# aws/sagemaker-xgboost-container

Hardware: NVIDIA H100
Metric: boosting rounds/sec (higher is better)
Workload: dtype int64

## Files before the change

### sagemaker-xgboost-container_b200/csrc/grow.cu

```cuda
#include "grow.h"
#include <algorithm>
#include <cmath>
#include <cstdlib>
#include <cstring>
#include "comm.h"

namespace b200 {

__global__ void pack_tree_kernel(TreeArrays t, const int* n_nodes, DevNode* out, int cap) {
  const int nn = *n_nodes;
  for (int i = blockIdx.x * blockDim.x + threadIdx.x; i < cap; i += gridDim.x * blockDim.x) {
    DevNode d;
    if (i < nn) { d.cond = t.split_cond[i]; d.left = t.left[i]; d.right = t.right[i]; d.fidx_dl = (unsigned)t.split_index[i] | ((unsigned)t.default_left[i] << 31); }
    else { d.cond = 0.f; d.left = -1; d.right = -1; d.fidx_dl = 0; }
    out[i] = d;
  }
}
__global__ void snapshot_h_kernel(const GH64* slot, long long* cache, size_t entries) {
  for (size_t e = (size_t)blockIdx.x * blockDim.x + threadIdx.x; e < entries; e += (size_t)gridDim.x * blockDim.x) cache[e] = slot[e].h;
}
__global__ void slot_from_cache_kernel(GH64* slot, const long long* cache, size_t entries) {
  for (size_t e = (size_t)blockIdx.x * blockDim.x + threadIdx.x; e < entries; e += (size_t)gridDim.x * blockDim.x) { GH64 v; v.g = 0; v.h = cache[e]; slot[e] = v; }
}
__global__ void gather_u32_kernel(const unsigned* src, const unsigned* idx, unsigned* dst, int64_t n) {
// ... 44 lines not shown
  if (lg_iters > 0) {
    max_nodes = 2 * lg_iters + 1; max_level_nodes = 2; region = 0;
    pool_slots = (size_t)lg_iters + kLgFirstFreeSlot;
  } else {
    max_nodes = (1 << (max_depth + 1)) - 1; max_level_nodes = 1 << (max_depth - 1); region = max_level_nodes;
    pool_slots = 2 * (size_t)region;
  }
  cap_nodes = (max_nodes + 15) & ~15;
  slot_stride = hist_slot_entries(ngroups, tw);
  const size_t partial_entries = hist_partial_entries(ngroups, tw, engine_num_sms(), max_level_nodes);
  const size_t pool_bytes = pool_slots * slot_stride * sizeof(GH64) + partial_entries * sizeof(int2);
  size_t free_b = 0, total_b = 0; cudaMemGetInfo(&free_b, &total_b);
  B200_CHECK(pool_bytes < free_b / 2 + hist_pool.n * sizeof(GH64) + hist_partials.n * sizeof(int2),
             "histogram pool for this max_depth / max_leaves / feature count does not fit in device memory");
  hist_pool.alloc(pool_slots * slot_stride);
  hist_partials.alloc(partial_entries);
  gpair.alloc((size_t)gp_stride * K + 512); gpair.zero(s); err.alloc(1); tree_index_dev.alloc(1);
  if (!leaf_scale.p) { leaf_scale.alloc(1); set_leaf_scale(1.0f); }
  root_h_cache.alloc(slot_stride);
  const bool routed = routes(lg_iters, max_depth);
  for (int i = 0; i < 2; ++i) { const size_t m = i == 0 || !routed ? (size_t)n : 0; ridx[i].alloc(m); gp[i].alloc(m); tl[i].alloc(tail_pos ? m : 0); }
  route_tiles = routed ? (unsigned)((n + kRouteTile - 1) / kRouteTile) : 0u;
  node_of_row.alloc(routed ? (size_t)n : 0);
  route_counts.alloc(routed && max_depth >= 2 ? ((size_t)1 << (max_depth - 2)) * route_tiles : 0);
  max_tiles = (unsigned)((n + kPartTile - 1) / kPartTile) + max_level_nodes + 1;
  scratch.alloc(3 * (size_t)max_level_nodes + 8);
  state_block.alloc(carve(gs, 0)); state_block.zero(s);
  carve(gs, (uintptr_t)state_block.p);
  tree_block.alloc(tree_block_bytes(cap_nodes));
  const TreeBlock tb = tree_block_layout(tree_block.p, cap_nodes);
  gs.n_nodes = tb.n_nodes; ta = tb.t; packed.alloc(cap_nodes);
  ic_path.alloc(n_ic ? (size_t)cap_nodes * F : 0); ic_allowed.alloc(n_ic ? (size_t)cap_nodes * F : 0);
  ic_sets.alloc((size_t)n_ic * F); ic_sets_host.clear();
  hist_configure();
  global_n = n;
  if (Comm::get().distributed()) {
    peer_reduce_setup({{hist_pool.p, hist_pool.n * sizeof(GH64)}, {state_block.p, state_block.n}}, s);
    DevBuf<double> dsum; dsum.alloc(1); double v = (double)n;
    CUDA_OK(cudaMemcpyAsync(dsum.p, &v, sizeof v, cudaMemcpyHostToDevice, s));
    Comm::get().allreduce_sum_f64(dsum.p, 1, s);
    CUDA_OK(cudaMemcpyAsync(&v, dsum.p, sizeof v, cudaMemcpyDeviceToHost, s));
    Comm::get().sync_stream(s);
    global_n = (int64_t)v;
  }
}

float* TreeBuilder::ensure_adaptive(int targets) {
// ... 129 lines not shown
  auto level_hist_args = [&](int set) {
    HistArgs ha = hist_args(bm, k);
    ha.ridx = ridx[set].p; ha.tail_pos = carry_tail ? tl[set].p : nullptr; ha.accumulate_sum = 0;
    ha.gpair = g_only ? nullptr : gp[set].p; ha.gpos = g_only ? reinterpret_cast<const float*>(gp[set].p) : nullptr;
    ha.rows_counter = profile ? prof_rows.p + 1 : nullptr;
    return ha;
  };
  launch_eval(eval_args(in, 0, in.mask), 1, s);
  for (int it = 0; it < in.lg_iters; ++it) {
    launch_apply_lossguide(apply_args(in, 0, 0, 0), it, s);
    const PartArgs pa = part_args(0, it == 0 ? kRootRows : 0, 1);
    timed(kProfPartition, [&] { launch_partition(pa, max_tiles, s); });
    launch_lg_copy_back(pa, ridx[0].p, gp[0].p, tl[0].p, max_tiles, s);
    launch_zero_build_slots(gs, hist_pool.p, slot_stride, 1, s);
    timed(kProfDeepHist, [&] { launch_hist_build(level_hist_args(0), num_sms, s); });
    if (dist) {
      launch_lg_stage(gs, hist_pool.p, slot_stride, 1, s);
      allreduce_hist(hist_pool.p + (size_t)kLgStageSlot * slot_stride, slot_stride * 2);
      launch_lg_stage(gs, hist_pool.p, slot_stride, 0, s);
    }
    launch_subtract(gs, hist_pool.p, slot_stride, 1, s);
    launch_eval(eval_args(in, 1, nullptr), 2, s);
  }
  for (int L = 0; L < D && in.lg_iters == 0; ++L) {
    const bool final_level = (L == D - 1);
    const int next_base = ((L + 1) & 1) * region, next_half = 1 << L;
    launch_apply(apply_args(in, L, next_base, next_half), s);
    if (final_level) break;
    if (routed) {
      RouteArgs ra{}; ra.gs = gs; ra.tree = ta; ra.bins_col = bm.bins_col; ra.n = bm.n; ra.node_of_row = node_of_row.p;
      ra.tile_counts = route_counts.p; ra.ntiles = route_tiles; ra.has_missing = bm.has_missing; ra.level = L;
      if (g_only) ra.g = g_dense(); else ra.gpair = gpair.p + (size_t)k * gp_stride;
      ra.g_only = g_only ? 1 : 0;
      ra.tail_row = carry_tail ? reinterpret_cast<const unsigned*>(bm.bins_tail) : nullptr;
      ra.ridx = ridx[0].p; ra.gp = gp[0].p; ra.tl = carry_tail ? tl[0].p : nullptr; ra.rows_counter = profile ? prof_rows.p + 2 : nullptr;
      timed(kProfPartition, [&] { launch_route(ra, s); });
    } else {
      PartArgs pa = part_args(L, L == 0 ? kRootRows : (L & 1) ^ 1, L & 1);
      pa.build_only = L == D - 2 ? 1 : 0;
      timed(kProfPartition, [&] { launch_partition(pa, max_tiles, s); });
    }
    CUDA_OK(cudaMemsetAsync(hist_pool.p + (size_t)next_base * slot_stride, 0, (size_t)next_half * slot_stride * sizeof(GH64), s));
    timed(kProfDeepHist, [&] { launch_hist_build(level_hist_args(routed ? 0 : L & 1), num_sms, s); });
    allreduce_hist(hist_pool.p + (size_t)next_base * slot_stride, (size_t)next_half * slot_stride * 2);
    launch_subtract(gs, hist_pool.p, slot_stride, next_half, s);
    launch_eval(eval_args(in, L + 1, in.mask ? in.mask + (size_t)(L + 1) * bm.F : nullptr), 1 << (L + 1), s);
  }
  const uint8_t* start = routed && D >= 2 ? node_of_row.p : nullptr;
  if (in.adaptive) {
    launch_locate_leaves(ta, gs.n_nodes, bm.bins_col, bm.n, bm.has_missing, start, g_only ? nullptr : gpair.p + (size_t)k * gp_stride, &adapt, s);
    SelectArgs sa{}; sa.values = in.resid; sa.seg = adapt.seg.p; sa.h = in.adaptive == 2 ? reinterpret_cast<const float*>(gpair.p + (size_t)k * gp_stride) + 1 : nullptr;
    sa.h_stride = 2; sa.scales = gs.scales; sa.n = bm.n; sa.nseg = max_leaves(); sa.alpha = (double)in.alpha;
    if (in.adaptive == 3) { sa.h = in.weight; sa.h_stride = 1; sa.scales = adapt.scales.p; }
    sa.leaf_nid = adapt.leaf_nid.p; sa.split_cond = ta.split_cond; sa.lr = in.p.eta;
    segmented_select(sa, &adapt, [&](unsigned long long* p, size_t cnt) { collective([p, cnt, s]() { Comm::get().allreduce_sum_i64(p, cnt, s); }); },
                     [&](unsigned* p, size_t cnt) { collective([p, cnt, s]() { Comm::get().allreduce_max_u32(p, cnt, s); }); }, s);
  }
  timed(kProfMargin, [&] { launch_update_margin(ta, gs.n_nodes, bm.bins_col, bm.n, bm.has_missing, start, in.margin, in.K, k, leaf_scale.p, s); });
  if (profile) prof_margin_rows += bm.n;
  pack_tree_kernel<<<(cap_nodes + 255) / 256, 256, 0, s>>>(ta, gs.n_nodes, packed.p, cap_nodes); ++g_kernel_launches;
  CUDA_OK(cudaGetLastError());
}
void TreeBuilder::end_segment() {
  cudaGraph_t graph = nullptr; cudaGraphExec_t exec = nullptr;
  CUDA_OK(cudaStreamEndCapture(engine_stream(), &graph));
  cudaError_t e = cudaGraphInstantiate(&exec, graph, 0);
  cudaGraphDestroy(graph);
  CUDA_OK(e);
// ... 166 lines not shown
```

### sagemaker-xgboost-container_b200/csrc/hist.cu

```cuda
#include <cuda.h>
#include <cstdlib>
#include <cstring>
#include <map>
#include <mutex>
#include <tuple>
#include <type_traits>
#include "engine.h"
#include "tree.h"

namespace b200 {

constexpr int kSuperRows = 32;
constexpr int kMinRowsPerCta = 4096;
constexpr int kSpillThresholdG = 1 << 25;
constexpr unsigned kSpillThresholdH = 1u << 26;
constexpr int kPlaneBytes = kGroupEntries * 4;
constexpr int kMaxSmem = 232448;
constexpr int kTeamWarps = 4, kTeams = 6, kRootRows = 16 * kTeamWarps;
constexpr int kRootConsumerWarps = kTeamWarps * kTeams;
constexpr int kRootProducerWarps = 3;
constexpr int kRootThreads = (kRootConsumerWarps + kRootProducerWarps) * 32;

template <int K, int N, typename F> __device__ __forceinline__ void static_for(F&& f) {
  if constexpr (K < N) { f(std::integral_constant<int, K>{}); static_for<K + 1, N>(f); }
// ... 567 lines not shown
      if ((it + 1) % iters_per_window == 0 && it + 1 < iters) {
        if (a.accumulate_sum && blockIdx.y == 0) { flush_node_sum(a.node_sum + nid, accG, accH, lane); accG = 0; accH = 0; }
        __syncthreads();
        spill_main<2>(smem, ng_here, out_main, false, threadIdx.x, NTHREADS);
        if (has_tail) spill_tail<2>(smem + NG * 2 * kGroupEntries, TWC, trep, out_tail, false, threadIdx.x, NTHREADS);
        __syncthreads();
      }
    }
    __syncthreads();
    if (a.partials) {
      int2* part = a.partials + (size_t)(blockIdx.x + b) * slot_entries;
      flush_partials<TWC, trep>(smem, smem + NG * 2 * kGroupEntries, ng_here, has_tail, part + (size_t)g0 * kGroupEntries,
                                part + (size_t)a.ngroups * kGroupEntries, out_tail, threadIdx.x, NTHREADS);
    } else {
      spill_main<2>(smem, ng_here, out_main, true, threadIdx.x, NTHREADS);
      if (has_tail) spill_tail<2>(smem + NG * 2 * kGroupEntries, TWC, trep, out_tail, true, threadIdx.x, NTHREADS);
    }
    __syncthreads();
    if (a.accumulate_sum && blockIdx.y == 0) flush_node_sum(a.node_sum + nid, accG, accH, lane);
    r0 = nend; ++b;
  }
}

__global__ void __launch_bounds__(256) hist_reduce_kernel(HistArgs a, unsigned C, unsigned sup) {
  const int nb = *a.build_count;
  if (nb <= 0) return;
  const unsigned T = a.build_prefix[nb];
  if (T == 0) return;
  unsigned ceff, chunk;
  gather_split(T, C, sup, ceff, chunk);
  const size_t slot_entries = (size_t)a.ngroups * kGroupEntries + (size_t)256 * a.tw;
  const size_t pairs = slot_entries / 2;
  for (size_t item = (size_t)blockIdx.x * blockDim.x + threadIdx.x; item < (size_t)nb * pairs; item += (size_t)gridDim.x * blockDim.x) {
    const int b = (int)(item / pairs);
    const size_t p = item - (size_t)b * pairs;
    const unsigned nbeg = a.build_prefix[b], nend = a.build_prefix[b + 1];
    if (nbeg == nend) continue;
    const unsigned x_lo = nbeg / chunk, nseg = (nend - 1) / chunk - x_lo + 1;
    const int4* src = reinterpret_cast<const int4*>(a.partials + (size_t)(x_lo + b) * slot_entries) + p;
    long long g0 = 0, h0 = 0, g1 = 0, h1 = 0;
    auto add = [&](const int4& v) { g0 += v.x; h0 += (unsigned)v.y; g1 += v.z; h1 += (unsigned)v.w; };
    unsigned s = 0;
    for (; s + 8 <= nseg; s += 8) {
      int4 v[8];
#pragma unroll
      for (int j = 0; j < 8; ++j) v[j] = __ldcs(src + (size_t)(s + j) * pairs);
#pragma unroll
      for (int j = 0; j < 8; ++j) add(v[j]);
    }
    for (; s < nseg; ++s) add(__ldcs(src + (size_t)s * pairs));
    longlong2* o = reinterpret_cast<longlong2*>(a.hist_pool + (size_t)a.hist_slot[a.build_nid[b]] * slot_entries + 2 * p);
    longlong2 e0 = o[0], e1 = o[1];
    e0.x += g0; e0.y += h0; e1.x += g1; e1.y += h1;
    o[0] = e0; o[1] = e1;
  }
}

static thread_local const char* g_last_kernel = "none";
const char* hist_last_kernel() { return g_last_kernel; }

static int chunks_for(int ngroups) { return (ngroups + 2) / 3; }
static int groups_per_chunk(int ngroups) { const int nc = chunks_for(ngroups); return (ngroups + nc - 1) / nc; }
static int gather_grid_x(int ngroups, int tw, int num_sms) {
  const int nchunks = chunks_for(ngroups);
  const int per_sm = groups_per_chunk(ngroups) > 1 ? 1 : (tw ? 1 : 3);
  return (num_sms * per_sm + nchunks - 1) / nchunks;
}
size_t hist_partial_entries(int ngroups, int tw, int num_sms, int max_build) {
  return ((size_t)gather_grid_x(ngroups, tw, num_sms) + (size_t)max_build) * hist_slot_entries(ngroups, tw);
}

static bool root_plan(int ngc, int tw, bool gonly, RootCfg* c) {
  const int PL = gonly ? 1 : 2;
  const unsigned main_b = (unsigned)ngc * PL * kPlaneBytes;
  const unsigned avail = kMaxSmem - 128  - 2 * 8 * 16 ;
  const unsigned stage = (unsigned)kRootRows * (32u * ngc + (gonly ? 4u : 8u) + tw);
  int trep = tw ? 32 / tw : 0;
// ... 56 lines not shown
void hist_configure() {
  static bool configured = false;
  if (configured) return;
  set_gather_attr<1, 0, 256>(); set_gather_attr<1, 4, 256>(); set_gather_attr<1, 8, 256>();
  set_gather_attr<2, 0, 768>(); set_gather_attr<2, 4, 768>(); set_gather_attr<2, 8, 768>();
  set_gather_attr<3, 0, 768>(); set_gather_attr<3, 4, 768>(); set_gather_attr<3, 8, 768>();
  CUDA_OK(cudaFuncSetAttribute(hist_root_kernel<false>, cudaFuncAttributeMaxDynamicSharedMemorySize, kMaxSmem));
  CUDA_OK(cudaFuncSetAttribute(hist_root_kernel<true>, cudaFuncAttributeMaxDynamicSharedMemorySize, kMaxSmem));
  configured = true;
}

template <int NG, int NT, bool GPAY>
static void launch_gather_tw(const HistArgs& a, int gx, int nchunks, cudaStream_t stream) {
  const int smem = NG * 2 * kPlaneBytes + (a.tw ? gather_tail_bytes(NG) : 0);
  if (a.tw == 0) hist_gather_kernel<NG, 0, NT, GPAY><<<dim3(gx, nchunks), NT, smem, stream>>>(a);
  else if (a.tw == 4) hist_gather_kernel<NG, 4, NT, GPAY><<<dim3(gx, nchunks), NT, smem, stream>>>(a);
  else hist_gather_kernel<NG, 8, NT, GPAY><<<dim3(gx, nchunks), NT, smem, stream>>>(a);
}
template <int NG, int NT>
static void launch_gather(const HistArgs& a, int gx, int nchunks, cudaStream_t stream) {
  if (a.gpos) launch_gather_tw<NG, NT, true>(a, gx, nchunks, stream); else launch_gather_tw<NG, NT, false>(a, gx, nchunks, stream);
}

void launch_hist_build(const HistArgs& a_in, int num_sms, cudaStream_t stream) {
  HistArgs a = a_in;
  const int nchunks = chunks_for(a.ngroups);
  a.ng_chunk = groups_per_chunk(a.ngroups);
  static const bool no_tma = getenv("B200XGB_NO_TMA") != nullptr;
  const bool gonly = a.g_only != 0;
  B200_CHECK(!gonly || a.gpos != nullptr, "hist: the G-only root pass reads the dense g (gpos)");
  if (a.ridx == nullptr && !no_tma && !a.force_gather && (a.gpos == nullptr || gonly)) {
    RootCfg c; CUtensorMap tm;
    if (root_plan(a.ng_chunk, a.tw, gonly, &c) && get_tensor_map(a.bins, a.n, a.row_stride, c.box_groups, kRootRows, &tm)) {
      const int gx = num_sms / nchunks > 0 ? num_sms / nchunks : 1;
      if (gonly) hist_root_kernel<true><<<dim3(gx, nchunks), kRootThreads, c.total, stream>>>(tm, a, c);
      else hist_root_kernel<false><<<dim3(gx, nchunks), kRootThreads, c.total, stream>>>(tm, a, c);
      g_last_kernel = gonly ? "hist_root_kernel<GONLY>" : "hist_root_kernel<GH>";
      ++g_kernel_launches;
      CUDA_OK(cudaGetLastError());
      return;
    }
  }
  B200_CHECK(!a.g_only || a.ridx == nullptr, "hist: G-only accumulation is a root-pass mode");
  B200_CHECK(!a.g_only, "hist: the G-only root pass needs the TMA kernel (tensor-map creation failed or B200XGB_NO_TMA is set)");
  static const bool red_flush = getenv("B200XGB_HIST_RED_FLUSH") != nullptr;
  if (red_flush) a.partials = nullptr;
  else B200_CHECK(a.partials != nullptr, "hist: the gathered passes need the builder's partial histograms");
  const int ng = a.ng_chunk;
  const int gx = gather_grid_x(a.ngroups, a.tw, num_sms);
  if (ng == 1) launch_gather<1, 256>(a, gx, nchunks, stream);
  else if (ng == 2) launch_gather<2, 768>(a, gx, nchunks, stream);
  else launch_gather<3, 768>(a, gx, nchunks, stream);
  g_last_kernel = "hist_gather_kernel";
  ++g_kernel_launches;
  CUDA_OK(cudaGetLastError());
  if (a.partials) {
    hist_reduce_kernel<<<num_sms * 8, 256, 0, stream>>>(a, (unsigned)gx, (unsigned)gather_super_rows(ng));
    ++g_kernel_launches;
    CUDA_OK(cudaGetLastError());
  }
}

}
```

### sagemaker-xgboost-container_b200/csrc/misc.cu

```cuda
#include <algorithm>
#include <cstdlib>
#include <utility>
#include "curve.h"
#include "elementwise.h"
#include "engine.h"
#include "inplace.h"
#include "misc.h"
#include "predict_tile.h"
#include "rng.h"
#include "transform.h"
#include "traverse.h"

namespace b200 {

__global__ void __launch_bounds__(256) gradient_kernel(GradArgs a) {
  float mg = 0.f, mh = 0.f;
  for (int64_t r = (int64_t)blockIdx.x * blockDim.x + threadIdx.x; r < a.n; r += (int64_t)gridDim.x * blockDim.x) {
    const float y = a.label[r];
    float w = a.weight ? a.weight[r] : 1.0f;
    const bool dropped = !row_sampled(a.seed, a.iter, (unsigned long long)(r + a.row_offset), a.subsample);
    if (a.objective == kSoftprob || a.objective == kSoftmax) {
      const int K = a.K;
      const float* m = a.margin ? a.margin + r * K : nullptr;
      float wmax = m ? m[0] : 0.f;
      for (int k = 1; k < K; ++k) wmax = fmaxf(wmax, m ? m[k] : 0.f);
      float wsum = 0.f;
      for (int k = 0; k < K; ++k) wsum += expf((m ? m[k] : 0.f) - wmax);
      int label = (int)y;
      if (label < 0 || label >= K) { *a.err = 2; label = 0; }
      for (int k = 0; k < K; ++k) {
        float pk = expf((m ? m[k] : 0.f) - wmax) / wsum;
        float h = fmaxf(2.0f * pk * (1.0f - pk) * w, 1e-16f);
        float g = (label == k ? pk - 1.0f : pk) * w;
        if (dropped) { g = 0.f; h = 0.f; }
        a.gpair[(int64_t)k * a.gp_stride + r] = make_float2(g, h);
        mg = fmaxf(mg, fabsf(g)); mh = fmaxf(mh, h);
      }
    } else {
      if (objective_is_reg_loss(a.objective) && y == 1.0f) w *= a.scale_pos_weight;
      float g, h;
      elementwise_gradient(a.objective, y, a.margin ? a.margin[r] : 0.f, a.aux, a.err, &g, &h);
      g *= w; h *= w;
      if (dropped) { g = 0.f; h = 0.f; }
      if (a.dense_g) reinterpret_cast<float*>(a.gpair)[r] = g; else a.gpair[r] = make_float2(g, h);
      mg = fmaxf(mg, fabsf(g)); mh = fmaxf(mh, h);
    }
  }
#pragma unroll
  for (int o = 16; o > 0; o >>= 1) { mg = fmaxf(mg, __shfl_xor_sync(0xffffffffu, mg, o)); mh = fmaxf(mh, __shfl_xor_sync(0xffffffffu, mh, o)); }
  __shared__ float sg[8], sh[8];
  if ((threadIdx.x & 31) == 0) { sg[threadIdx.x >> 5] = mg; sh[threadIdx.x >> 5] = mh; }
  __syncthreads();
  if (threadIdx.x == 0) {
    for (int w = 1; w < 8; ++w) { mg = fmaxf(mg, sg[w]); mh = fmaxf(mh, sh[w]); }
    if (a.absmax) { atomicMax(a.absmax, __float_as_uint(mg)); atomicMax(a.absmax + 1, __float_as_uint(mh)); }
  }
}

__global__ void __launch_bounds__(256) sample_gpair_kernel(SampleArgs a) {
  float mg = 0.f, mh = 0.f;
  for (int64_t r = (int64_t)blockIdx.x * blockDim.x + threadIdx.x; r < a.n; r += (int64_t)gridDim.x * blockDim.x) {
    const bool keep = rng_uniform(a.seed, a.stream, (unsigned long long)(r + a.row_offset)) < a.subsample;
    for (int k = 0; k < a.K; ++k) {
      const float2 v = keep ? a.src[(int64_t)k * a.gp_stride + r] : make_float2(0.f, 0.f);
      a.dst[(int64_t)k * a.gp_stride + r] = v;
      mg = fmaxf(mg, fabsf(v.x)); mh = fmaxf(mh, v.y);
    }
  }
// ... 303 lines not shown
```

### sagemaker-xgboost-container_b200/csrc/tree.cu

```cuda
#include <algorithm>
#include <type_traits>
#include "engine.h"
#include "rng.h"
#include "split_math.h"
#include "tree.h"

namespace b200 {


__device__ __forceinline__ void interaction_children(const ApplyArgs& a, int nid, int f, int Lc, int Rc) {
  if (a.node_allowed == nullptr) return;
  const size_t F = (size_t)a.F;
  unsigned char* pl = a.node_path + (size_t)Lc * F; unsigned char* pr = a.node_path + (size_t)Rc * F;
  unsigned char* al = a.node_allowed + (size_t)Lc * F; unsigned char* ar = a.node_allowed + (size_t)Rc * F;
  const unsigned char* pp = a.node_path + (size_t)nid * F;
  for (int j = 0; j < a.F; ++j) { const unsigned char v = (pp[j] || j == f) ? 1 : 0; pl[j] = v; pr[j] = v; al[j] = v; ar[j] = v; }
  for (int s = 0; s < a.n_ic_sets; ++s) {
    const unsigned char* set = a.ic_sets + (size_t)s * F;
    bool relevant = true;
    for (int j = 0; j < a.F && relevant; ++j) if (pl[j] && !set[j]) relevant = false;
    if (relevant) for (int j = 0; j < a.F; ++j) if (set[j]) { al[j] = 1; ar[j] = 1; }
  }
}

// ... 568 lines not shown
    const unsigned id = (ids[q >> 2] >> (8 * (q & 3))) & 0xffu;
    const PackedNode p = s_node[id];
    const unsigned child = p.left == 0xffff ? id : (goes_left(p, byte[q], a.has_missing) ? p.left : p.left + 1u);
    out[q >> 2] |= child << (8 * (q & 3));
    const unsigned c = r < a.n ? s_bidx[child] : 0xffu;
    const unsigned m = __match_any_sync(0xffffffffu, c);
    if (c != 0xffu && lane == __ffs(m) - 1) atomicAdd(&s_cnt[c], (unsigned)__popc(m));
  }
#pragma unroll
  for (int j = 0; j < kRuns; ++j) {
    const int64_t r = r0 + j * 1024;
    if (a.level > 0 && out[j] == ids[j]) continue;
    if (r + 4 <= a.n) *reinterpret_cast<unsigned*>(a.node_of_row + r) = out[j];
    else for (int e = 0; e < 4; ++e) if (r + e < a.n) a.node_of_row[r + e] = (uint8_t)(out[j] >> (8 * e));
  }
  __syncthreads();
  for (int c = threadIdx.x; c < nb; c += blockDim.x) a.tile_counts[(size_t)c * a.ntiles + blockIdx.x] = s_cnt[c];
  if (a.rows_counter && threadIdx.x == 0) {
    const int64_t t0 = (int64_t)blockIdx.x * kRouteTile;
    atomicAdd(a.rows_counter, (unsigned long long)(a.n - t0 < (int64_t)kRouteTile ? a.n - t0 : (int64_t)kRouteTile));
  }
}

__global__ void __launch_bounds__(1024) route_scan_kernel(RouteArgs a) {
  __shared__ unsigned s_run[1024], s_tmp[33];
  const int c = blockIdx.x;
  if (c >= *a.gs.build_count) return;
  unsigned* cnt = a.tile_counts + (size_t)c * a.ntiles;
  const unsigned per = (a.ntiles + blockDim.x - 1) / blockDim.x, t0 = threadIdx.x * per, t1 = min(t0 + per, a.ntiles);
  unsigned sum = 0;
#pragma unroll 8
  for (unsigned t = t0; t < t1; ++t) sum += cnt[t];
  s_run[threadIdx.x] = sum;
  __syncthreads();
  const unsigned tot = block_exclusive_scan(s_run, s_run, (int)blockDim.x, s_tmp);
  unsigned run = s_run[threadIdx.x];
#pragma unroll 8
  for (unsigned t = t0; t < t1; ++t) { const unsigned v = cnt[t]; cnt[t] = run; run += v; }
  if (threadIdx.x == 0) a.gs.seg_count[a.gs.build_nid[c]] = tot;
}

constexpr int kWarpRows = kRouteTile / 8, kWarpSteps = kWarpRows / 32;
template <bool GONLY, bool TL>
__global__ void __launch_bounds__(256, 4) scatter_kernel(RouteArgs a) {
  typedef typename std::conditional<GONLY, float, float2>::type Pay;
  __shared__ unsigned char s_bidx[kRouteMaxNodes];
  __shared__ unsigned s_start[kRouteMaxBuild];
  __shared__ unsigned s_local[kRouteMaxBuild + 1];
  __shared__ unsigned s_dst[kRouteMaxBuild];
  __shared__ unsigned s_wofs[8][kRouteMaxBuild];
  __shared__ unsigned s_rid[kRouteTile];
  __shared__ Pay s_gp[kRouteTile];
  __shared__ unsigned s_tl[TL ? kRouteTile : 1];
  __shared__ unsigned char s_ch[kRouteTile];
  const GrowState& gs = a.gs;
  const int nb = *gs.build_count;
  if (nb == 0) { if (blockIdx.x == 0 && threadIdx.x == 0) gs.build_prefix[0] = 0; return; }
  stage_route_tables(a, nullptr, s_bidx, nb);
  if (threadIdx.x < nb) s_start[threadIdx.x] = gs.seg_count[gs.build_nid[threadIdx.x]];
  __syncthreads();
  if (threadIdx.x == 0) {
    unsigned run = 0;
    for (int c = 0; c < nb; ++c) {
      const unsigned t = s_start[c]; s_start[c] = run;
      if (blockIdx.x == 0) { gs.build_prefix[c] = run; gs.seg_begin[gs.build_nid[c]] = run; }
      run += t;
    }
    if (blockIdx.x == 0) gs.build_prefix[nb] = run;
  }
  const int lane = threadIdx.x & 31, warp = threadIdx.x >> 5;
  const unsigned lanes_below = (1u << lane) - 1u;
  for (unsigned tile = blockIdx.x; tile < a.ntiles; tile += gridDim.x) {
    const int64_t rw = (int64_t)tile * kRouteTile + warp * kWarpRows + lane;
    unsigned ck[kWarpSteps];
#pragma unroll
    for (int it = 0; it < kWarpSteps; ++it) { const int64_t r = rw + it * 32; ck[it] = r < a.n ? a.node_of_row[r] : kRouteMaxNodes - 1; }
    const unsigned toff = threadIdx.x < nb ? a.tile_counts[(size_t)threadIdx.x * a.ntiles + tile] : 0u;
    __syncthreads();
    for (int i = threadIdx.x; i < 8 * kRouteMaxBuild; i += blockDim.x) s_wofs[i / kRouteMaxBuild][i % kRouteMaxBuild] = 0;
    __syncthreads();
#pragma unroll
    for (int it = 0; it < kWarpSteps; ++it) {
      const unsigned c = s_bidx[ck[it]];
      const unsigned m = __match_any_sync(0xffffffffu, c);
      const unsigned before = c != 0xffu ? s_wofs[warp][c] : 0u;
      __syncwarp();
      if (c != 0xffu && lane == __ffs(m) - 1) s_wofs[warp][c] = before + __popc(m);
      __syncwarp();
      ck[it] = c << 16 | (before + __popc(m & lanes_below));
    }
    __syncthreads();
    if (threadIdx.x < nb) {
      unsigned t = 0;
      for (int w = 0; w < 8; ++w) t += s_wofs[w][threadIdx.x];
      s_local[threadIdx.x + 1] = t;
    }
    __syncthreads();
    if (threadIdx.x == 0) { s_local[0] = 0; for (int c = 0; c < nb; ++c) s_local[c + 1] += s_local[c]; }
    __syncthreads();
    if (threadIdx.x < nb) {
// ... 106 lines not shown
void launch_lg_copy_back(const PartArgs& a, unsigned* ridx_dst, void* gp_dst, unsigned* tl_dst, unsigned max_tiles, cudaStream_t s) {
  const unsigned grid = max_tiles < 1184u ? max_tiles : 1184u;
  if (a.g_only) lg_copy_back_kernel<float><<<grid, 256, 0, s>>>(a, ridx_dst, static_cast<float*>(gp_dst), tl_dst);
  else lg_copy_back_kernel<float2><<<grid, 256, 0, s>>>(a, ridx_dst, static_cast<float2*>(gp_dst), tl_dst);
  ++g_kernel_launches; CUDA_OK(cudaGetLastError());
}
void launch_zero_build_slots(const GrowState& gs, GH64* pool, size_t slot_entries, int max_build, cudaStream_t s) {
  dim3 grid(max_build, (unsigned)((slot_entries + 1023) / 1024)); zero_build_slots_kernel<<<grid, 256, 0, s>>>(gs, pool, slot_entries); ++g_kernel_launches; CUDA_OK(cudaGetLastError());
}
void launch_lg_stage(const GrowState& gs, GH64* pool, size_t slot_entries, int to_stage, cudaStream_t s) {
  lg_stage_kernel<<<(unsigned)((slot_entries + 1023) / 1024), 256, 0, s>>>(gs, pool, slot_entries, to_stage); ++g_kernel_launches; CUDA_OK(cudaGetLastError());
}
void launch_apply(const ApplyArgs& a, cudaStream_t s) { apply_kernel<<<1, 256, 0, s>>>(a); ++g_kernel_launches; CUDA_OK(cudaGetLastError()); }
void launch_partition(const PartArgs& a, unsigned max_tiles, cudaStream_t s) {
  CUDA_OK(cudaMemsetAsync(a.gs.tile_desc, 0, sizeof(unsigned long long) * ((size_t)max_tiles + 1), s));
  const bool tl = a.tl_cur != nullptr;
  if (a.g_only) { if (tl) part_kernel<true, true><<<max_tiles, 256, 0, s>>>(a); else part_kernel<true, false><<<max_tiles, 256, 0, s>>>(a); }
  else { if (tl) part_kernel<false, true><<<max_tiles, 256, 0, s>>>(a); else part_kernel<false, false><<<max_tiles, 256, 0, s>>>(a); }
  ++g_kernel_launches; CUDA_OK(cudaGetLastError());
}
void launch_route(const RouteArgs& a, cudaStream_t s) {
  if (a.ntiles == 0) return;
  route_kernel<<<a.ntiles, 256, 0, s>>>(a); ++g_kernel_launches; CUDA_OK(cudaGetLastError());
  route_scan_kernel<<<1u << a.level, 1024, 0, s>>>(a); ++g_kernel_launches; CUDA_OK(cudaGetLastError());
  const bool tl = a.tail_row != nullptr;
  const unsigned grid = std::min(a.ntiles, 4u * (unsigned)engine_num_sms());
  if (a.g_only) { if (tl) scatter_kernel<true, true><<<grid, 256, 0, s>>>(a); else scatter_kernel<true, false><<<grid, 256, 0, s>>>(a); }
  else { if (tl) scatter_kernel<false, true><<<grid, 256, 0, s>>>(a); else scatter_kernel<false, false><<<grid, 256, 0, s>>>(a); }
  ++g_kernel_launches; CUDA_OK(cudaGetLastError());
}
void launch_update_margin(const TreeArrays& t, const int* n_nodes, const uint8_t* bins_col, int64_t n, int has_missing, const uint8_t* node_of_row,
                          float* margin, int K, int k, const float* leaf_scale, cudaStream_t s) {
  if (n == 0) return;
  update_margin_kernel<<<(unsigned)((n + 1023) / 1024), 256, 0, s>>>(t, n_nodes, bins_col, n, has_missing, node_of_row, margin, K, k, leaf_scale);
  ++g_kernel_launches; CUDA_OK(cudaGetLastError());
}
void launch_subtract(const GrowState& gs, GH64* pool, size_t slot_entries, int max_build, cudaStream_t s) {
  dim3 grid(max_build, (unsigned)((slot_entries + 1023) / 1024)); subtract_kernel<<<grid, 256, 0, s>>>(gs, pool, slot_entries); ++g_kernel_launches; CUDA_OK(cudaGetLastError());
}

}
```

### sagemaker-xgboost-container_b200/csrc/tree.h

```cpp
#pragma once
#include "engine.h"

namespace b200 {

constexpr unsigned kPartTile = 2048;

struct TrainParamDev {
  float eta, lambda, alpha, gamma, min_child_weight, max_delta_step;
  int max_depth, max_leaves;
};

struct EvalArgs {
  const GH64* hist_pool; GrowState gs; const int* cut_ptrs; const unsigned char* feat_mask;
  TrainParamDev p; int F, ngroups, tw, ntail, has_missing, level, max_level_nodes;
  const int* monotone;
  const unsigned char* node_allowed;
  float colsample_bynode; unsigned seed; const int* tree_index;
};

struct ApplyArgs {
  GrowState gs; TreeArrays tree; const int* cut_ptrs; const float* cut_vals; const float* min_vals;
  TrainParamDev p; unsigned* scratch; int nblocks , level, max_level_nodes, next_base, next_half;
  const int* monotone;
  unsigned char* node_path; unsigned char* node_allowed; const unsigned char* ic_sets; int n_ic_sets, F;
};

struct PartArgs {
  GrowState gs; TreeArrays tree; const uint8_t* bins_col; int64_t n; const unsigned* ridx_cur; unsigned* ridx_next;
  const void* gp_cur; void* gp_next; int g_only;
  const unsigned* tl_cur; unsigned* tl_next;
  int has_missing, level, max_level_nodes;
  int build_only;
  unsigned long long* rows_counter;
};

constexpr int kRouteMaxDepth = 7;
constexpr unsigned kRouteTile = 2048;
constexpr int kRouteMaxNodes = 256;
constexpr int kRouteMaxBuild = 1 << (kRouteMaxDepth - 2);
struct RouteArgs {
  GrowState gs; TreeArrays tree; const uint8_t* bins_col; int64_t n;
  uint8_t* node_of_row;
  unsigned* tile_counts;
  unsigned ntiles; int has_missing, level;
  const float* g; const float2* gpair; int g_only; const unsigned* tail_row;
  unsigned* ridx; void* gp; unsigned* tl;
  unsigned long long* rows_counter;
};

struct HistArgs {
  const uint8_t* bins;
  const uint8_t* bins_tail;
  const unsigned* tail_pos;
  int64_t n;
  int row_stride;
  const uint8_t* bins_gather;
  int gather_stride;
  int tail_in_gather;
  int tw;
  const float2* gpair;
  const float* gpos;
  const unsigned* ridx;
  const int* build_count;
  const int* build_nid;
  const unsigned* build_prefix;
  const unsigned* seg_begin;
  const int* hist_slot;
  const float* scales;
  GH64* hist_pool;
  GH64* node_sum;
  int2* partials;
  int ngroups;
  int ng_chunk;
  int accumulate_sum;
  int g_only;
  int window_rows;
  int force_gather;
  unsigned long long* rows_counter;
};

constexpr int kLgRootSlot = 0, kLgStageSlot = 1, kLgFirstFreeSlot = 2;
void launch_apply_lossguide(const ApplyArgs& a, int iter, cudaStream_t s);
void launch_lg_copy_back(const PartArgs& a, unsigned* ridx_dst, void* gp_dst, unsigned* tl_dst, unsigned max_tiles, cudaStream_t s);
void launch_zero_build_slots(const GrowState& gs, GH64* pool, size_t slot_entries, int max_build, cudaStream_t s);
void launch_lg_stage(const GrowState& gs, GH64* pool, size_t slot_entries, int to_stage, cudaStream_t s);
void launch_hist_build(const HistArgs& a, int num_sms, cudaStream_t stream);
size_t hist_partial_entries(int ngroups, int tw, int num_sms, int max_build);
void hist_configure();
const char* hist_last_kernel();
void launch_init_tree(const GrowState& gs, const TreeArrays& t, unsigned n, cudaStream_t s);
void launch_scales(const GrowState& gs, int grad_bits, cudaStream_t s);
void launch_eval(const EvalArgs& a, int max_nodes_level, cudaStream_t s);
void launch_apply(const ApplyArgs& a, cudaStream_t s);
void launch_partition(const PartArgs& a, unsigned max_tiles, cudaStream_t s);
void launch_route(const RouteArgs& a, cudaStream_t s);
void launch_update_margin(const TreeArrays& t, const int* n_nodes, const uint8_t* bins_col, int64_t n, int has_missing, const uint8_t* node_of_row,
                          float* margin, int K, int k, const float* leaf_scale, cudaStream_t s);
void launch_subtract(const GrowState& gs, GH64* pool, size_t slot_entries, int max_build, cudaStream_t s);

}
```

Before: 107.2.

## Fuse sibling subtraction and slot zeroing into hist reduce, parallelize route scan

Folds the sibling-histogram subtraction and the next level's slot zeroing into the partial-histogram reduce kernel, which removes a separate subtract launch and a memset per level. The route scan now runs as a 2D grid over tile chunks and writes offsets to a separate buffer, replacing the old single block per node. The gradient kernel batches four rows per thread to expose more memory-level parallelism. A profiling script is added. The fused path writes parent and sibling slots from the reduce, which relies on correct slot indexing, and it needs twice the route-count memory.

```diff
diff --git a/microbench/level_chain_profile.py b/microbench/level_chain_profile.py
--- /dev/null
+++ b/microbench/level_chain_profile.py
@@ -0,0 +1,132 @@
+#!/usr/bin/env python
+import argparse
+import collections
+import json
+import os
+import sys
+import tempfile
+
+ROOT = os.path.dirname(os.path.dirname(os.path.abspath(__file__)))
+sys.path.insert(0, ROOT)
+
+MARK = "FillFunctor"
+
+
+def short_name(name):
+    n = name.split("(")[0]
+    n = n.split("<")[0]
+    return n.split(" ")[-1].split("::")[-1] or name
+
+
+def device_activities(trace_path):
+    with open(trace_path) as f:
+        ev = json.load(f)["traceEvents"]
+    out = []
+    for e in ev:
+        cat = e.get("cat", "")
+        if cat not in ("kernel", "gpu_memset", "gpu_memcpy") or "dur" not in e:
+            continue
+        name = e["name"]
+        if MARK in name:
+            name = MARK
+        elif cat == "gpu_memset":
+            name = "memset"
+        elif cat == "gpu_memcpy":
+            name = "memcpy"
+        else:
+            name = short_name(name)
+        out.append((float(e["ts"]), float(e["dur"]), name))
+    out.sort()
+    return out
+
+
+def split_rounds(acts):
+    rounds, cur = [], None
+    for a in acts:
+        if a[2] == MARK:
+            if cur is not None:
+                rounds.append(cur)
+            cur = []
+        elif cur is not None:
+            cur.append(a)
+    if cur:
+        rounds.append(cur)
+    return rounds
+
+
+def summarize(acts):
+    kernels = collections.OrderedDict()
+    gaps = collections.OrderedDict()
+    total_gap = 0.0
+    for i, (ts, dur, name) in enumerate(acts):
+        k = kernels.setdefault(name, {"count": 0, "device_us": 0.0})
+        k["count"] += 1
+        k["device_us"] += dur
+        if i > 0:
+            g = max(0.0, ts - (acts[i - 1][0] + acts[i - 1][1]))
+            gaps[name] = gaps.get(name, 0.0) + g
+            total_gap += g
+    span = acts[-1][0] + acts[-1][1] - acts[0][0] if acts else 0.0
+    return {"span_us": span, "busy_us": sum(a[1] for a in acts), "gap_us": total_gap, "launches": len(acts),
+            "kernels": kernels, "gap_before_us": gaps}
+
+
+def main():
+    ap = argparse.ArgumentParser()
+    ap.add_argument("--rows", type=int, default=50_000_000)
+    ap.add_argument("--cols", type=int, default=100)
+    ap.add_argument("--max-depth", type=int, default=6)
+    ap.add_argument("--objective", default="reg:squarederror")
+    ap.add_argument("--warmup", type=int, default=5)
+    ap.add_argument("--rounds", type=int, default=3)
+    ap.add_argument("--out", default="")
+    a = ap.parse_args()
+    import torch
+    from torch.profiler import ProfilerActivity, profile
+    import bench
+    import sagemaker_xgboost_container_b200 as xgb
+    be = xgb.get_backend()
+    dev = torch.device("cuda", 0)
+    ba = argparse.Namespace(rows=a.rows, cols=a.cols, seed=43, objective=a.objective, num_class=0)
+    X, y = bench.gen_shard(ba, 0, a.rows, dev)
+    d = xgb.DMatrix(X, label=y.cpu().numpy())
+    del X
+    torch.cuda.empty_cache()
+    params = bench.params_of(argparse.Namespace(objective=a.objective, max_depth=a.max_depth, max_bin=256, num_class=0))
+    b = xgb.Booster(params, [d])
+    it = 0
+    for _ in range(a.warmup):
+        b.update(d, it); it += 1
+    mark = torch.zeros(1, device=dev)
+    be.synchronize(); torch.cuda.synchronize()
+    with tempfile.TemporaryDirectory() as tmp:
+        with profile(activities=[ProfilerActivity.CUDA]) as prof:
+            for r in range(a.rounds):
+                mark.fill_(float(r)); torch.cuda.synchronize()
+                b.update(d, it); it += 1
+                be.synchronize(); torch.cuda.synchronize()
+            mark.fill_(-1.0); torch.cuda.synchronize()
+        path = os.path.join(tmp, "trace.json")
+        prof.export_chrome_trace(path)
+        rounds = split_rounds(device_activities(path))
+    if len(rounds) != a.rounds:
+        raise RuntimeError("found %d rounds in the trace, expected %d" % (len(rounds), a.rounds))
+    per_round = [summarize(r) for r in rounds]
+    names = list(per_round[0]["kernels"].keys())
+    table = {n: {"count": sum(p["kernels"].get(n, {}).get("count", 0) for p in per_round) / a.rounds,
+                 "device_us": sum(p["kernels"].get(n, {}).get("device_us", 0.0) for p in per_round) / a.rounds,
+                 "gap_before_us": sum(p["gap_before_us"].get(n, 0.0) for p in per_round) / a.rounds} for n in names}
+    out = {"gpu": torch.cuda.get_device_name(dev), "rows": a.rows, "cols": a.cols, "objective": a.objective, "max_depth": a.max_depth,
+           "rounds": a.rounds, "mean_per_round": {"span_us": sum(p["span_us"] for p in per_round) / a.rounds,
+                                                  "busy_us": sum(p["busy_us"] for p in per_round) / a.rounds,
+                                                  "gap_us": sum(p["gap_us"] for p in per_round) / a.rounds,
+                                                  "launches": sum(p["launches"] for p in per_round) / a.rounds, "kernels": table},
+           "per_round": per_round}
+    print(json.dumps(out["mean_per_round"]), flush=True)
+    if a.out:
+        with open(a.out, "w") as f:
+            json.dump(out, f, indent=1)
+
+
+if __name__ == "__main__":
+    main()
diff --git a/sagemaker-xgboost-container_b200/csrc/grow.cu b/sagemaker-xgboost-container_b200/csrc/grow.cu
--- a/sagemaker-xgboost-container_b200/csrc/grow.cu
+++ b/sagemaker-xgboost-container_b200/csrc/grow.cu
@@ -90,7 +90,7 @@
   for (int i = 0; i < 2; ++i) { const size_t m = i == 0 || !routed ? (size_t)n : 0; ridx[i].alloc(m); gp[i].alloc(m); tl[i].alloc(tail_pos ? m : 0); }
   route_tiles = routed ? (unsigned)((n + kRouteTile - 1) / kRouteTile) : 0u;
   node_of_row.alloc(routed ? (size_t)n : 0);
-  route_counts.alloc(routed && max_depth >= 2 ? ((size_t)1 << (max_depth - 2)) * route_tiles : 0);
+  route_counts.alloc(routed && max_depth >= 2 ? 2 * ((size_t)1 << (max_depth - 2)) * route_tiles : 0);
   max_tiles = (unsigned)((n + kPartTile - 1) / kPartTile) + max_level_nodes + 1;
   scratch.alloc(3 * (size_t)max_level_nodes + 8);
   state_block.alloc(carve(gs, 0)); state_block.zero(s);
@@ -266,6 +266,8 @@
     launch_subtract(gs, hist_pool.p, slot_stride, 1, s);
     launch_eval(eval_args(in, 1, nullptr), 2, s);
   }
+  static const bool separate_subtract = getenv("B200XGB_SEPARATE_SUBTRACT") != nullptr;
+  const bool fused = !dist && hist_reduces_partials() && !separate_subtract;
   for (int L = 0; L < D && in.lg_iters == 0; ++L) {
     const bool final_level = (L == D - 1);
     const int next_base = ((L + 1) & 1) * region, next_half = 1 << L;
@@ -273,7 +275,7 @@
     if (final_level) break;
     if (routed) {
       RouteArgs ra{}; ra.gs = gs; ra.tree = ta; ra.bins_col = bm.bins_col; ra.n = bm.n; ra.node_of_row = node_of_row.p;
-      ra.tile_counts = route_counts.p; ra.ntiles = route_tiles; ra.has_missing = bm.has_missing; ra.level = L;
+      ra.tile_counts = route_counts.p; ra.tile_offsets = route_counts.p + route_counts.n / 2; ra.ntiles = route_tiles; ra.has_missing = bm.has_missing; ra.level = L;
       if (g_only) ra.g = g_dense(); else ra.gpair = gpair.p + (size_t)k * gp_stride;
       ra.g_only = g_only ? 1 : 0;
       ra.tail_row = carry_tail ? reinterpret_cast<const unsigned*>(bm.bins_tail) : nullptr;
@@ -284,10 +286,15 @@
       pa.build_only = L == D - 2 ? 1 : 0;
       timed(kProfPartition, [&] { launch_partition(pa, max_tiles, s); });
     }
-    CUDA_OK(cudaMemsetAsync(hist_pool.p + (size_t)next_base * slot_stride, 0, (size_t)next_half * slot_stride * sizeof(GH64), s));
-    timed(kProfDeepHist, [&] { launch_hist_build(level_hist_args(routed ? 0 : L & 1), num_sms, s); });
+    if (!fused || L == 0) CUDA_OK(cudaMemsetAsync(hist_pool.p + (size_t)next_base * slot_stride, 0, (size_t)next_half * slot_stride * sizeof(GH64), s));
+    HistArgs ha = level_hist_args(routed ? 0 : L & 1);
+    if (fused) {
+      ha.fuse_subtract = 1; ha.build_sub_nid = gs.build_sub_nid; ha.build_parent_slot = gs.build_parent_slot;
+      if (L + 2 < D) { ha.zero_first = (L & 1) * region; ha.zero_count = 2 << L; }
+    }
+    timed(kProfDeepHist, [&] { launch_hist_build(ha, num_sms, s); });
     allreduce_hist(hist_pool.p + (size_t)next_base * slot_stride, (size_t)next_half * slot_stride * 2);
-    launch_subtract(gs, hist_pool.p, slot_stride, next_half, s);
+    if (!fused) launch_subtract(gs, hist_pool.p, slot_stride, next_half, s);
     launch_eval(eval_args(in, L + 1, in.mask ? in.mask + (size_t)(L + 1) * bm.F : nullptr), 1 << (L + 1), s);
   }
   const uint8_t* start = routed && D >= 2 ? node_of_row.p : nullptr;
diff --git a/sagemaker-xgboost-container_b200/csrc/hist.cu b/sagemaker-xgboost-container_b200/csrc/hist.cu
--- a/sagemaker-xgboost-container_b200/csrc/hist.cu
+++ b/sagemaker-xgboost-container_b200/csrc/hist.cu
@@ -613,21 +613,42 @@
   }
 }
 
+constexpr int kMaxZeroSlots = 1 << (kMaxDepth - 2);
 __global__ void __launch_bounds__(256) hist_reduce_kernel(HistArgs a, unsigned C, unsigned sup) {
+  __shared__ unsigned s_parent[kMaxZeroSlots / 32];
   const int nb = *a.build_count;
   if (nb <= 0) return;
   const unsigned T = a.build_prefix[nb];
-  if (T == 0) return;
-  unsigned ceff, chunk;
-  gather_split(T, C, sup, ceff, chunk);
+  if (T == 0 && !a.fuse_subtract) return;
+  unsigned ceff = 1, chunk = 1;
+  if (T > 0) gather_split(T, C, sup, ceff, chunk);
   const size_t slot_entries = (size_t)a.ngroups * kGroupEntries + (size_t)256 * a.tw;
   const size_t pairs = slot_entries / 2;
-  for (size_t item = (size_t)blockIdx.x * blockDim.x + threadIdx.x; item < (size_t)nb * pairs; item += (size_t)gridDim.x * blockDim.x) {
+  const int zc = a.fuse_subtract ? a.zero_count : 0;
+  if (zc > 0) {
+    for (int i = threadIdx.x; i < (zc + 31) / 32; i += blockDim.x) s_parent[i] = 0u;
+    __syncthreads();
+    for (int b = threadIdx.x; b < nb; b += blockDim.x) {
+      const unsigned z = (unsigned)(a.build_parent_slot[b] - a.zero_first);
+      if (z < (unsigned)zc) atomicOr(&s_parent[z >> 5], 1u << (z & 31));
+    }
+    __syncthreads();
+  }
+  const size_t items = (size_t)nb * pairs, all_items = items + (size_t)zc * pairs;
+  for (size_t item = (size_t)blockIdx.x * blockDim.x + threadIdx.x; item < all_items; item += (size_t)gridDim.x * blockDim.x) {
+    if (item >= items) {
+      const int z = (int)((item - items) / pairs);
+      if (s_parent[z >> 5] & (1u << (z & 31))) continue;
+      const size_t p = item - items - (size_t)z * pairs;
+      longlong2* o = reinterpret_cast<longlong2*>(a.hist_pool + (size_t)(a.zero_first + z) * slot_entries + 2 * p);
+      o[0] = make_longlong2(0, 0); o[1] = make_longlong2(0, 0);
+      continue;
+    }
     const int b = (int)(item / pairs);
     const size_t p = item - (size_t)b * pairs;
     const unsigned nbeg = a.build_prefix[b], nend = a.build_prefix[b + 1];
-    if (nbeg == nend) continue;
-    const unsigned x_lo = nbeg / chunk, nseg = (nend - 1) / chunk - x_lo + 1;
+    if (nbeg == nend && !a.fuse_subtract) continue;
+    const unsigned x_lo = nbeg / chunk, nseg = nbeg == nend ? 0u : (nend - 1) / chunk - x_lo + 1;
     const int4* src = reinterpret_cast<const int4*>(a.partials + (size_t)(x_lo + b) * slot_entries) + p;
     long long g0 = 0, h0 = 0, g1 = 0, h1 = 0;
     auto add = [&](const int4& v) { g0 += v.x; h0 += (unsigned)v.y; g1 += v.z; h1 += (unsigned)v.w; };
@@ -644,6 +665,13 @@
     longlong2 e0 = o[0], e1 = o[1];
     e0.x += g0; e0.y += h0; e1.x += g1; e1.y += h1;
     o[0] = e0; o[1] = e1;
+    if (a.fuse_subtract) {
+      longlong2* par = reinterpret_cast<longlong2*>(a.hist_pool + (size_t)a.build_parent_slot[b] * slot_entries + 2 * p);
+      longlong2* sib = reinterpret_cast<longlong2*>(a.hist_pool + (size_t)a.hist_slot[a.build_sub_nid[b]] * slot_entries + 2 * p);
+      const longlong2 p0 = par[0], p1 = par[1];
+      sib[0] = make_longlong2(p0.x - e0.x, p0.y - e0.y); sib[1] = make_longlong2(p1.x - e1.x, p1.y - e1.y);
+      if ((unsigned)(a.build_parent_slot[b] - a.zero_first) < (unsigned)zc) { par[0] = make_longlong2(0, 0); par[1] = make_longlong2(0, 0); }
+    }
   }
 }
 
@@ -746,6 +774,11 @@
   if (a.gpos) launch_gather_tw<NG, NT, true>(a, gx, nchunks, stream); else launch_gather_tw<NG, NT, false>(a, gx, nchunks, stream);
 }
 
+bool hist_reduces_partials() {
+  static const bool red_flush = getenv("B200XGB_HIST_RED_FLUSH") != nullptr;
+  return !red_flush;
+}
+
 void launch_hist_build(const HistArgs& a_in, int num_sms, cudaStream_t stream) {
   HistArgs a = a_in;
   const int nchunks = chunks_for(a.ngroups);
@@ -767,9 +800,9 @@
   }
   B200_CHECK(!a.g_only || a.ridx == nullptr, "hist: G-only accumulation is a root-pass mode");
   B200_CHECK(!a.g_only, "hist: the G-only root pass needs the TMA kernel (tensor-map creation failed or B200XGB_NO_TMA is set)");
-  static const bool red_flush = getenv("B200XGB_HIST_RED_FLUSH") != nullptr;
-  if (red_flush) a.partials = nullptr;
+  if (!hist_reduces_partials()) a.partials = nullptr;
   else B200_CHECK(a.partials != nullptr, "hist: the gathered passes need the builder's partial histograms");
+  B200_CHECK(!a.fuse_subtract || (a.partials != nullptr && a.zero_count <= kMaxZeroSlots), "hist: the sibling subtraction is fused into the partial-slot reduce only");
   const int ng = a.ng_chunk;
   const int gx = gather_grid_x(a.ngroups, a.tw, num_sms);
   if (ng == 1) launch_gather<1, 256>(a, gx, nchunks, stream);
diff --git a/sagemaker-xgboost-container_b200/csrc/misc.cu b/sagemaker-xgboost-container_b200/csrc/misc.cu
--- a/sagemaker-xgboost-container_b200/csrc/misc.cu
+++ b/sagemaker-xgboost-container_b200/csrc/misc.cu
@@ -13,13 +13,15 @@
 
 namespace b200 {
 
-__global__ void __launch_bounds__(256) gradient_kernel(GradArgs a) {
+constexpr int kGradRows = 4;
+__global__ void __launch_bounds__(256, 4) gradient_kernel(GradArgs a) {
   float mg = 0.f, mh = 0.f;
-  for (int64_t r = (int64_t)blockIdx.x * blockDim.x + threadIdx.x; r < a.n; r += (int64_t)gridDim.x * blockDim.x) {
-    const float y = a.label[r];
-    float w = a.weight ? a.weight[r] : 1.0f;
-    const bool dropped = !row_sampled(a.seed, a.iter, (unsigned long long)(r + a.row_offset), a.subsample);
-    if (a.objective == kSoftprob || a.objective == kSoftmax) {
+  const int64_t stride = (int64_t)gridDim.x * blockDim.x;
+  if (a.objective == kSoftprob || a.objective == kSoftmax) {
+    for (int64_t r = (int64_t)blockIdx.x * blockDim.x + threadIdx.x; r < a.n; r += stride) {
+      const float y = a.label[r];
+      const float w = a.weight ? a.weight[r] : 1.0f;
+      const bool dropped = !row_sampled(a.seed, a.iter, (unsigned long long)(r + a.row_offset), a.subsample);
       const int K = a.K;
       const float* m = a.margin ? a.margin + r * K : nullptr;
       float wmax = m ? m[0] : 0.f;
@@ -36,14 +38,31 @@
         a.gpair[(int64_t)k * a.gp_stride + r] = make_float2(g, h);
         mg = fmaxf(mg, fabsf(g)); mh = fmaxf(mh, h);
       }
-    } else {
-      if (objective_is_reg_loss(a.objective) && y == 1.0f) w *= a.scale_pos_weight;
-      float g, h;
-      elementwise_gradient(a.objective, y, a.margin ? a.margin[r] : 0.f, a.aux, a.err, &g, &h);
-      g *= w; h *= w;
-      if (dropped) { g = 0.f; h = 0.f; }
-      if (a.dense_g) reinterpret_cast<float*>(a.gpair)[r] = g; else a.gpair[r] = make_float2(g, h);
-      mg = fmaxf(mg, fabsf(g)); mh = fmaxf(mh, h);
+    }
+  } else {
+    for (int64_t r0 = (int64_t)blockIdx.x * blockDim.x + threadIdx.x; r0 < a.n; r0 += kGradRows * stride) {
+      float y[kGradRows], p[kGradRows], w[kGradRows];
+#pragma unroll
+      for (int j = 0; j < kGradRows; ++j) {
+        const int64_t r = r0 + j * stride;
+        const bool in = r < a.n;
+        y[j] = in ? a.label[r] : 0.f;
+        p[j] = in && a.margin ? a.margin[r] : 0.f;
+        w[j] = in && a.weight ? a.weight[r] : 1.0f;
+      }
+#pragma unroll
+      for (int j = 0; j < kGradRows; ++j) {
+        const int64_t r = r0 + j * stride;
+        if (r >= a.n) break;
+        const bool dropped = !row_sampled(a.seed, a.iter, (unsigned long long)(r + a.row_offset), a.subsample);
+        if (objective_is_reg_loss(a.objective) && y[j] == 1.0f) w[j] *= a.scale_pos_weight;
+        float g, h;
+        elementwise_gradient(a.objective, y[j], p[j], a.aux, a.err, &g, &h);
+        g *= w[j]; h *= w[j];
+        if (dropped) { g = 0.f; h = 0.f; }
+        if (a.dense_g) reinterpret_cast<float*>(a.gpair)[r] = g; else a.gpair[r] = make_float2(g, h);
+        mg = fmaxf(mg, fabsf(g)); mh = fmaxf(mh, h);
+      }
     }
   }
 #pragma unroll
diff --git a/sagemaker-xgboost-container_b200/csrc/tree.cu b/sagemaker-xgboost-container_b200/csrc/tree.cu
--- a/sagemaker-xgboost-container_b200/csrc/tree.cu
+++ b/sagemaker-xgboost-container_b200/csrc/tree.cu
@@ -614,22 +614,37 @@
   }
 }
 
-__global__ void __launch_bounds__(1024) route_scan_kernel(RouteArgs a) {
-  __shared__ unsigned s_run[1024], s_tmp[33];
-  const int c = blockIdx.x;
+constexpr unsigned kScanChunk = 1024;
+__global__ void __launch_bounds__(kScanChunk) route_scan_kernel(RouteArgs a) {
+  constexpr int kWarps = kScanChunk / 32;
+  __shared__ unsigned s_warp[kWarps];
+  const int c = blockIdx.y;
   if (c >= *a.gs.build_count) return;
-  unsigned* cnt = a.tile_counts + (size_t)c * a.ntiles;
-  const unsigned per = (a.ntiles + blockDim.x - 1) / blockDim.x, t0 = threadIdx.x * per, t1 = min(t0 + per, a.ntiles);
-  unsigned sum = 0;
-#pragma unroll 8
-  for (unsigned t = t0; t < t1; ++t) sum += cnt[t];
-  s_run[threadIdx.x] = sum;
-  __syncthreads();
-  const unsigned tot = block_exclusive_scan(s_run, s_run, (int)blockDim.x, s_tmp);
-  unsigned run = s_run[threadIdx.x];
-#pragma unroll 8
-  for (unsigned t = t0; t < t1; ++t) { const unsigned v = cnt[t]; cnt[t] = run; run += v; }
-  if (threadIdx.x == 0) a.gs.seg_count[a.gs.build_nid[c]] = tot;
+  const unsigned* cnt = a.tile_counts + (size_t)c * a.ntiles;
+  const unsigned t0 = blockIdx.x * kScanChunk, t = t0 + threadIdx.x;
+  const int lane = threadIdx.x & 31, warp = threadIdx.x >> 5;
+  const unsigned v = t < a.ntiles ? cnt[t] : 0u;
+  unsigned before = 0;
+#pragma unroll 16
+  for (unsigned u = threadIdx.x; u < t0; u += kScanChunk) before += cnt[u];
+  unsigned x = v;
+#pragma unroll
+  for (int o = 16; o > 0; o >>= 1) before += __shfl_xor_sync(0xffffffffu, before, o);
+#pragma unroll
+  for (int o = 1; o < 32; o <<= 1) { const unsigned y = __shfl_up_sync(0xffffffffu, x, o); if (lane >= o) x += y; }
+  if (lane == 0) s_warp[warp] = before;
+  __syncthreads();
+  unsigned carry = 0;
+#pragma unroll
+  for (int w = 0; w < kWarps; ++w) carry += s_warp[w];
+  __syncthreads();
+  if (lane == 31) s_warp[warp] = x;
+  __syncthreads();
+  unsigned below = 0, tot = 0;
+#pragma unroll
+  for (int w = 0; w < kWarps; ++w) { const unsigned u = s_warp[w]; below += w < warp ? u : 0u; tot += u; }
+  if (t < a.ntiles) a.tile_offsets[(size_t)c * a.ntiles + t] = carry + below + x - v;
+  if (blockIdx.x == gridDim.x - 1 && threadIdx.x == 0) a.gs.seg_count[a.gs.build_nid[c]] = carry + tot;
 }
 
 constexpr int kWarpRows = kRouteTile / 8, kWarpSteps = kWarpRows / 32;
@@ -667,7 +682,7 @@
     unsigned ck[kWarpSteps];
 #pragma unroll
     for (int it = 0; it < kWarpSteps; ++it) { const int64_t r = rw + it * 32; ck[it] = r < a.n ? a.node_of_row[r] : kRouteMaxNodes - 1; }
-    const unsigned toff = threadIdx.x < nb ? a.tile_counts[(size_t)threadIdx.x * a.ntiles + tile] : 0u;
+    const unsigned toff = threadIdx.x < nb ? a.tile_offsets[(size_t)threadIdx.x * a.ntiles + tile] : 0u;
     __syncthreads();
     for (int i = threadIdx.x; i < 8 * kRouteMaxBuild; i += blockDim.x) s_wofs[i / kRouteMaxBuild][i % kRouteMaxBuild] = 0;
     __syncthreads();
@@ -820,7 +835,8 @@
 void launch_route(const RouteArgs& a, cudaStream_t s) {
   if (a.ntiles == 0) return;
   route_kernel<<<a.ntiles, 256, 0, s>>>(a); ++g_kernel_launches; CUDA_OK(cudaGetLastError());
-  route_scan_kernel<<<1u << a.level, 1024, 0, s>>>(a); ++g_kernel_launches; CUDA_OK(cudaGetLastError());
+  const dim3 scan_grid((a.ntiles + kScanChunk - 1) / kScanChunk, 1u << a.level);
+  route_scan_kernel<<<scan_grid, kScanChunk, 0, s>>>(a); ++g_kernel_launches; CUDA_OK(cudaGetLastError());
   const bool tl = a.tail_row != nullptr;
   const unsigned grid = std::min(a.ntiles, 4u * (unsigned)engine_num_sms());
   if (a.g_only) { if (tl) scatter_kernel<true, true><<<grid, 256, 0, s>>>(a); else scatter_kernel<true, false><<<grid, 256, 0, s>>>(a); }
diff --git a/sagemaker-xgboost-container_b200/csrc/tree.h b/sagemaker-xgboost-container_b200/csrc/tree.h
--- a/sagemaker-xgboost-container_b200/csrc/tree.h
+++ b/sagemaker-xgboost-container_b200/csrc/tree.h
@@ -42,6 +42,7 @@
   GrowState gs; TreeArrays tree; const uint8_t* bins_col; int64_t n;
   uint8_t* node_of_row;
   unsigned* tile_counts;
+  unsigned* tile_offsets;
   unsigned ntiles; int has_missing, level;
   const float* g; const float2* gpair; int g_only; const unsigned* tail_row;
   unsigned* ridx; void* gp; unsigned* tl;
@@ -70,6 +71,9 @@
   GH64* hist_pool;
   GH64* node_sum;
   int2* partials;
+  const int* build_sub_nid; const int* build_parent_slot;
+  int fuse_subtract;
+  int zero_first, zero_count;
   int ngroups;
   int ng_chunk;
   int accumulate_sum;
@@ -85,6 +89,7 @@
 void launch_zero_build_slots(const GrowState& gs, GH64* pool, size_t slot_entries, int max_build, cudaStream_t s);
 void launch_lg_stage(const GrowState& gs, GH64* pool, size_t slot_entries, int to_stage, cudaStream_t s);
 void launch_hist_build(const HistArgs& a, int num_sms, cudaStream_t stream);
+bool hist_reduces_partials();
 size_t hist_partial_entries(int ngroups, int tw, int num_sms, int max_build);
 void hist_configure();
 const char* hist_last_kernel();
```

Measured after the change: 109.7 (median of 6 runs). 1.02x the previous value.
